# hygenie1228/PoseRisk_RELEASE

Measured on AMD Instinct MI355X. Metric: frames/sec (224x224 crops) through SPIN ResNet-50 + regressor + SMPL LBS + REBA/RULA, higher is better.
Workload: dtype f32; 1 GPU; configs[1]: batch=64 random 224x224 crops per GPU, ResNet-50+SMPL fp32; global_batch=64, batches_in_flight=3, hipgraph_replay=False, exchange=none, dist_world_size=1

## Files before the change

### poserisk_release_amd/csrc/conv_fused.hip

```cpp
#include <cstdlib>

#include "conv_igemm.h"
#include "kernel_vocab.h"

namespace pr {
namespace {

constexpr int BK = kConvBK;

struct FArgs {
  const float* x;
  const float* w2;
  const float* bias2;
  const float* w3;
  const float* bias3;
  const float* res;
  float* y;
  unsigned x_bytes, w2_bytes, w3_bytes;
  int H, W, Cin, log2Cin, HoWo, M, nk, N3, relu3;
};

constexpr int kStage = 2 * 64 * 128;
constexpr int kT2 = 0;
constexpr int kRing = 2 * 8192;
constexpr int kLds = 2 * kStage;

__global__ __launch_bounds__(256, 5) void conv3x3_conv1x1_f32(const FArgs a) {
#if defined(__HIP_DEVICE_COMPILE__)
  extern __shared__ __attribute__((aligned(16))) char smem[];
  const int nb = gridDim.x, bid = blockIdx.x;
  const int tile_m = xcd_contiguous_block<int>(bid, nb);
  const int m0 = tile_m * 64;
  const int tid = threadIdx.x, lane = tid & 63;
  const int wave = __builtin_amdgcn_readfirstlane(tid >> 6);
  const int wm = wave >> 1, wn = wave & 1;

  const int q = PR_DMA_SWIZZLE_SLOT(lane, wave);
  const auto xsrc = make_rsrc(a.x, (int)a.x_bytes);
  const auto w2src = make_rsrc(a.w2, (int)a.w2_bytes);
  const auto w3src = make_rsrc(a.w3, (int)a.w3_bytes);
  int a_base[2], a_hi0[2], a_wi0[2];
  unsigned b2_off[2], b3_off[2];
  const int K2 = a.nk * BK;
#pragma unroll
  for (int i = 0; i < 2; ++i) {
    const int r = 8 * (wave + 4 * i) + (lane >> 3);
    const int m = m0 + r;
    if (m < a.M) {
      const int img = m / a.HoWo, rem = m - img * a.HoWo;
      const int ho = rem / a.W, wo = rem - ho * a.W;
      a_hi0[i] = ho - 1;
      a_wi0[i] = wo - 1;
      a_base[i] = (((img * a.H + a_hi0[i]) * a.W + a_wi0[i]) * a.Cin + q * 4) * 4;
    } else {
      a_hi0[i] = -(1 << 28);
      a_wi0[i] = 0;
      a_base[i] = (int)kOOB;
    }
    b2_off[i] = (unsigned)((r * K2 + q * 4) * 4);
    b3_off[i] = (unsigned)((r * 64 + q * 4) * 4);
  }

  auto issue = [&](int kt, int buf) {
    char* stage = smem + buf * kStage;
    const int k0 = kt * BK;
    const int tap = k0 >> a.log2Cin, ci0 = k0 & (a.Cin - 1);
    const int kh = tap / 3, kw = tap - kh * 3;
    const int koff = ((kh * a.W + kw) * a.Cin + ci0) * 4;
#pragma unroll
    for (int i = 0; i < 2; ++i) {
      const bool ok = (unsigned)(a_hi0[i] + kh) < (unsigned)a.H && (unsigned)(a_wi0[i] + kw) < (unsigned)a.W;
      __builtin_amdgcn_raw_ptr_buffer_load_lds(xsrc, (lds_void*)(stage + (wave + 4 * i) * 1024), 16,
                                               ok ? (unsigned)(a_base[i] + koff) : kOOB, 0, 0, 0);
    }
#pragma unroll
    for (int i = 0; i < 2; ++i)
      __builtin_amdgcn_raw_ptr_buffer_load_lds(w2src, (lds_void*)(stage + 8192 + (wave + 4 * i) * 1024), 16, b2_off[i],
                                               kt * 128, 0, 0);
  };
  auto issue3 = [&](int s) {
    char* stage = smem + kRing + (s & 1) * 8192;
    const int soff = ((s >> 1) * 64 * 64 + (s & 1) * BK) * 4;
#pragma unroll
    for (int i = 0; i < 2; ++i)
      __builtin_amdgcn_raw_ptr_buffer_load_lds(w3src, (lds_void*)(stage + (wave + 4 * i) * 1024), 16, b3_off[i], soff, 0, 0);
  };

  const int frow = lane & 31, fh = lane >> 5, fsw = (frow >> 1) & 7;
  int foff[BK / 8];
#pragma unroll
  for (int kk = 0; kk < BK / 8; ++kk) foff[kk] = frow * 128 + (((2 * kk + fh) ^ fsw) << 4);

  f32x16 acc;
#pragma unroll
  for (int e = 0; e < 16; ++e) acc[e] = 0.f;
  auto compute = [&](const char* Ab, const char* Bb) {
    f32x4 af[BK / 8], bf[BK / 8];
#pragma unroll
    for (int kk = 0; kk < BK / 8; ++kk) {
      af[kk] = *reinterpret_cast<const f32x4*>(Ab + foff[kk]);
      bf[kk] = *reinterpret_cast<const f32x4*>(Bb + foff[kk]);
    }
    __builtin_amdgcn_sched_barrier(0);
#pragma unroll
    for (int kk = 0; kk < BK / 8; ++kk)
#pragma unroll
      for (int j = 0; j < 4; ++j) acc = __builtin_amdgcn_mfma_f32_32x32x2f32(af[kk][j], bf[kk][j], acc, 0, 0, 0);
  };

  issue(0, 0);
  for (int kt = 0; kt < a.nk; ++kt) {
    asm volatile("s_waitcnt vmcnt(0)" ::: "memory");
    __builtin_amdgcn_s_barrier();
    asm volatile("" ::: "memory");
    if (kt + 1 < a.nk) issue(kt + 1, (kt + 1) & 1);
    const char* st = smem + (kt & 1) * kStage;
    compute(st + wm * 32 * 128, st + 8192 + wn * 32 * 128);
  }

  __syncthreads();
  issue3(0);
  {
    const int c = lane & 31;
    const float b2 = a.bias2[wn * 32 + c];
    char* t2 = smem + kT2 + wn * 8192;
#pragma unroll
    for (int e = 0; e < 16; ++e) {
      const int r = wm * 32 + 4 * (lane >> 5) + (e & 3) + 8 * (e >> 2);
      const float v = fmaxf(acc[e] + b2, 0.f);
      *reinterpret_cast<float*>(t2 + r * 128 + ((((c >> 2) ^ ((r >> 1) & 7))) << 4) + (c & 3) * 4) = v;
    }
  }

  const int nsteps = (a.N3 >> 6) * 2;
  float rfrag[16];
  const int col_l = lane & 31, row_h = 4 * (lane >> 5);
  const int yz_bytes = a.M * a.N3 * 4;
  const auto rsrc = make_rsrc(a.res ? a.res : a.y, yz_bytes);
  const auto ysrc = make_rsrc(a.y, yz_bytes);
  const int frag_off = ((m0 + wm * 32 + row_h) * a.N3 + wn * 32 + col_l) * 4;
  const int mlim = a.M - (m0 + wm * 32 + row_h);
  for (int s = 0; s < nsteps; ++s) {
    asm volatile("s_waitcnt vmcnt(0) lgkmcnt(0)" ::: "memory");
    __builtin_amdgcn_s_barrier();
    asm volatile("" ::: "memory");
    if (s + 1 < nsteps) issue3(s + 1);
    const int n0 = (s >> 1) * 64;
    if ((s & 1) == 0) {
#pragma unroll
      for (int e = 0; e < 16; ++e) acc[e] = 0.f;
      if (a.res) {
#pragma unroll
        for (int e = 0; e < 16; ++e)
          rfrag[e] = __builtin_bit_cast(float, __builtin_amdgcn_raw_buffer_load_b32(
                                                   rsrc, (e & 3) + 8 * (e >> 2) < mlim ? frag_off : (int)kOOB,
                                                   (n0 + ((e & 3) + 8 * (e >> 2)) * a.N3) * 4, 0));
      }
    }
    compute(smem + kT2 + (s & 1) * 8192 + wm * 32 * 128, smem + kRing + (s & 1) * 8192 + wn * 32 * 128);
    if (s & 1) {
      const float b3 = a.bias3[n0 + wn * 32 + col_l];
#pragma unroll
      for (int e = 0; e < 16; ++e) {
        float v = acc[e] + b3;
        if (a.res) v += rfrag[e];
        if (a.relu3) v = fmaxf(v, 0.f);
        __builtin_amdgcn_raw_buffer_store_b32(__builtin_bit_cast(unsigned, v), ysrc,
                                              (e & 3) + 8 * (e >> 2) < mlim ? frag_off : (int)kOOB,
                                              (n0 + ((e & 3) + 8 * (e >> 2)) * a.N3) * 4, 0);
      }
    }
  }
#endif
}

struct PArgs {
  const float* x;
  const float* x2;
  const float* w;
  const float* bias;
  const float* res;
  float* y;
  unsigned x_bytes, x2_bytes, w_bytes;
  int M, N, K, nk, nk1, HoWo, Wo, H2, W2, Cin2, stride2;
  int chunks, nsplit, relu;
};

template <bool DUAL>
__global__ __launch_bounds__(256, 3) void conv1x1_panel_f32(const PArgs a) {
#if defined(__HIP_DEVICE_COMPILE__)
  extern __shared__ __attribute__((aligned(16))) char smem[];
  const int nb = gridDim.x, bid = blockIdx.x;
  const int item = xcd_contiguous_block<int>(bid, nb);
  const int panel = item / a.nsplit, part = item - panel * a.nsplit;
  const int m0 = panel * 64, nbase = part * a.chunks * 64;
  const int tid = threadIdx.x, lane = tid & 63;
  const int wave = __builtin_amdgcn_readfirstlane(tid >> 6);
  const int wm = wave >> 1, wn = wave & 1;
  const int q = PR_DMA_SWIZZLE_SLOT(lane, wave);
  const auto xsrc = make_rsrc(a.x, (int)a.x_bytes);
  [[maybe_unused]] const auto x2src = make_rsrc(DUAL ? a.x2 : a.x, DUAL ? (int)a.x2_bytes : 0);
  const auto wsrc = make_rsrc(a.w, (int)a.w_bytes);
  char* ring = smem + a.nk * 8192;

  const int K1 = a.nk1 * BK;
  unsigned b_off[2];
#pragma unroll
  for (int i = 0; i < 2; ++i) {
    const int r = 8 * (wave + 4 * i) + (lane >> 3);
    const int m = m0 + r;
    unsigned base = kOOB, base2 = kOOB;
    if (m < a.M) {
      base = (unsigned)((m * K1 + q * 4) * 4);
      if (DUAL) {
        const int img = m / a.HoWo, rem = m - img * a.HoWo;
        const int ho = rem / a.Wo, wo = rem - ho * a.Wo;
        base2 = (unsigned)((((img * a.H2 + ho * a.stride2) * a.W2 + wo * a.stride2) * a.Cin2 + q * 4) * 4);
      }
    }
    for (int kt = 0; kt < a.nk; ++kt) {
      lds_void* dst = (lds_void*)(smem + kt * 8192 + (wave + 4 * i) * 1024);
      if (DUAL && kt >= a.nk1) __builtin_amdgcn_raw_ptr_buffer_load_lds(x2src, dst, 16, base2, (kt - a.nk1) * 128, 0, 0);
      else __builtin_amdgcn_raw_ptr_buffer_load_lds(xsrc, dst, 16, base, kt * 128, 0, 0);
    }
    b_off[i] = (unsigned)((r * a.K + q * 4) * 4);
  }
  auto issue_w = [&](int chunk, int kt, int buf) {
    const int soff = ((nbase + chunk * 64) * a.K + kt * BK) * 4;
#pragma unroll
    for (int i = 0; i < 2; ++i)
      __builtin_amdgcn_raw_ptr_buffer_load_lds(wsrc, (lds_void*)(ring + buf * 8192 + (wave + 4 * i) * 1024), 16, b_off[i],
                                               soff, 0, 0);
  };
  issue_w(0, 0, 0);

  const int frow = lane & 31, fh = lane >> 5, fsw = (frow >> 1) & 7;
  int foff[BK / 8];
#pragma unroll
  for (int kk = 0; kk < BK / 8; ++kk) foff[kk] = frow * 128 + (((2 * kk + fh) ^ fsw) << 4);
  f32x16 acc;
  float rfrag[16];
  const int col_l = lane & 31, row_h = 4 * (lane >> 5);
  const int yz_bytes = a.M * a.N * 4;
  const auto rsrc = make_rsrc(a.res ? a.res : a.y, yz_bytes);
  const auto ysrc = make_rsrc(a.y, yz_bytes);
  const int frag_off = ((m0 + wm * 32 + row_h) * a.N + nbase + wn * 32 + col_l) * 4;
  const int mlim = a.M - (m0 + wm * 32 + row_h);

  int chunk = 0, kt = 0;
  const int nsteps = a.chunks * a.nk;
  for (int s = 0; s < nsteps; ++s) {
    asm volatile("s_waitcnt vmcnt(0)" ::: "memory");
    __builtin_amdgcn_s_barrier();
    asm volatile("" ::: "memory");
    {
      int nchunk = chunk, nkt = kt + 1;
      if (nkt == a.nk) { nkt = 0; ++nchunk; }
      if (s + 1 < nsteps) issue_w(nchunk, nkt, (s + 1) & 1);
    }
    const int n0 = chunk * 64;
    if (kt == 0) {
#pragma unroll
      for (int e = 0; e < 16; ++e) acc[e] = 0.f;
      if (a.res) {
#pragma unroll
        for (int e = 0; e < 16; ++e)
          rfrag[e] = __builtin_bit_cast(float, __builtin_amdgcn_raw_buffer_load_b32(
                                                   rsrc, (e & 3) + 8 * (e >> 2) < mlim ? frag_off : (int)kOOB,
                                                   (n0 + ((e & 3) + 8 * (e >> 2)) * a.N) * 4, 0));
      }
    }
    {
      const char* Ab = smem + kt * 8192 + wm * 32 * 128;
      const char* Bb = ring + (s & 1) * 8192 + wn * 32 * 128;
      f32x4 af[BK / 8], bf[BK / 8];
#pragma unroll
      for (int kk = 0; kk < BK / 8; ++kk) {
        af[kk] = *reinterpret_cast<const f32x4*>(Ab + foff[kk]);
        bf[kk] = *reinterpret_cast<const f32x4*>(Bb + foff[kk]);
      }
      __builtin_amdgcn_sched_barrier(0);
#pragma unroll
      for (int kk = 0; kk < BK / 8; ++kk)
#pragma unroll
        for (int j = 0; j < 4; ++j) acc = __builtin_amdgcn_mfma_f32_32x32x2f32(af[kk][j], bf[kk][j], acc, 0, 0, 0);
    }
    if (kt == a.nk - 1) {
      const float b = a.bias ? a.bias[nbase + n0 + wn * 32 + col_l] : 0.f;
#pragma unroll
      for (int e = 0; e < 16; ++e) {
        float v = acc[e] + b;
        if (a.res) v += rfrag[e];
        if (a.relu) v = fmaxf(v, 0.f);
        __builtin_amdgcn_raw_buffer_store_b32(__builtin_bit_cast(unsigned, v), ysrc,
                                              (e & 3) + 8 * (e >> 2) < mlim ? frag_off : (int)kOOB,
                                              (n0 + ((e & 3) + 8 * (e >> 2)) * a.N) * 4, 0);
      }
      kt = 0;
      ++chunk;
    } else {
      ++kt;
    }
  }
#endif
}


struct FArgsB {
  const unsigned short* x;
  const unsigned short* w2;
  const float* bias2;
  const unsigned short* w3;
  const float* bias3;
  const unsigned short* res;
  unsigned short* y;
  unsigned x_bytes, w2_bytes, w3_bytes;
  int H, W, Cin, log2Cin, HoWo, M, nk, N3, relu3;
};

constexpr int kBStage = 2 * 64 * 128;
constexpr int kBT2 = 0;
constexpr int kBRing = 8192;
constexpr int kBCt = 8192 + 16384;
constexpr int kBLds = kBCt + 64 * 64 * 4;

__device__ inline unsigned short f2bf(float f) {
  const __bf16 h = (__bf16)f;
  return __builtin_bit_cast(unsigned short, h);
}

__global__ __launch_bounds__(256, 4) void conv3x3_conv1x1_bf16(const FArgsB a) {
#if defined(__HIP_DEVICE_COMPILE__)
  extern __shared__ __attribute__((aligned(16))) char smem[];
  constexpr int BKB = 64;
  const int nb = gridDim.x, bid = blockIdx.x;
  const int tile_m = xcd_contiguous_block<int>(bid, nb);
  const int m0 = tile_m * 64;
  const int tid = threadIdx.x, lane = tid & 63;
  const int wave = __builtin_amdgcn_readfirstlane(tid >> 6);
  const int wm = wave >> 1, wn = wave & 1;
  const int q = PR_DMA_SWIZZLE_SLOT(lane, wave);
  const auto xsrc = make_rsrc(a.x, (int)a.x_bytes);
  const auto w2src = make_rsrc(a.w2, (int)a.w2_bytes);
  const auto w3src = make_rsrc(a.w3, (int)a.w3_bytes);
  int a_base[2], a_hi0[2], a_wi0[2];
  unsigned b2_off[2], b3_off[2];
  const int K2 = a.nk * BKB;
#pragma unroll
  for (int i = 0; i < 2; ++i) {
    const int r = 8 * (wave + 4 * i) + (lane >> 3);
    const int m = m0 + r;
    if (m < a.M) {
      const int img = m / a.HoWo, rem = m - img * a.HoWo;
      const int ho = rem / a.W, wo = rem - ho * a.W;
      a_hi0[i] = ho - 1;
      a_wi0[i] = wo - 1;
      a_base[i] = (((img * a.H + a_hi0[i]) * a.W + a_wi0[i]) * a.Cin + q * 8) * 2;
    } else {
      a_hi0[i] = -(1 << 28);
      a_wi0[i] = 0;
      a_base[i] = (int)kOOB;
    }
    b2_off[i] = (unsigned)((r * K2 + q * 8) * 2);
    b3_off[i] = (unsigned)((r * 64 + q * 8) * 2);
  }
  auto issue = [&](int kt, int buf) {
    char* stage = smem + buf * kBStage;
    const int tap = kt % 9, ci0 = (kt / 9) * BKB;
    const int kh = tap / 3, kw = tap - kh * 3;
    const int koff = ((kh * a.W + kw) * a.Cin + ci0) * 2;
#pragma unroll
    for (int i = 0; i < 2; ++i) {
      const bool ok = (unsigned)(a_hi0[i] + kh) < (unsigned)a.H && (unsigned)(a_wi0[i] + kw) < (unsigned)a.W;
      __builtin_amdgcn_raw_ptr_buffer_load_lds(xsrc, (lds_void*)(stage + (wave + 4 * i) * 1024), 16,
                                               ok ? (unsigned)(a_base[i] + koff) : kOOB, 0, 0, 0);
    }
#pragma unroll
    for (int i = 0; i < 2; ++i)
      __builtin_amdgcn_raw_ptr_buffer_load_lds(w2src, (lds_void*)(stage + 8192 + (wave + 4 * i) * 1024), 16, b2_off[i],
                                               kt * 128, 0, 0);
  };
  auto issue3 = [&](int nc) {
    char* stage = smem + kBRing + (nc & 1) * 8192;
#pragma unroll
    for (int i = 0; i < 2; ++i)
      __builtin_amdgcn_raw_ptr_buffer_load_lds(w3src, (lds_void*)(stage + (wave + 4 * i) * 1024), 16, b3_off[i],
                                               nc * 64 * 64 * 2, 0, 0);
  };

  const int frow = lane & 31, fh = lane >> 5, fsw = (frow >> 1) & 7;
  int foff[4];
#pragma unroll
  for (int kk = 0; kk < 4; ++kk) foff[kk] = frow * 128 + (((2 * kk + fh) ^ fsw) << 4);
  f32x16 acc;
#pragma unroll
  for (int e = 0; e < 16; ++e) acc[e] = 0.f;
  auto compute = [&](const char* Ab, const char* Bb) {
    bf16x8 af[4], bf[4];
#pragma unroll
    for (int kk = 0; kk < 4; ++kk) {
      af[kk] = *reinterpret_cast<const bf16x8*>(Ab + foff[kk]);
      bf[kk] = *reinterpret_cast<const bf16x8*>(Bb + foff[kk]);
    }
#pragma unroll
    for (int kk = 0; kk < 4; ++kk) acc = mfma_bf16_step(af[kk], bf[kk], acc);
  };

  issue(0, 0);
  for (int kt = 0; kt < a.nk; ++kt) {
    asm volatile("s_waitcnt vmcnt(0)" ::: "memory");
    __builtin_amdgcn_s_barrier();
    asm volatile("" ::: "memory");
    if (kt + 1 < a.nk) issue(kt + 1, (kt + 1) & 1);
    const char* st = smem + (kt & 1) * kBStage;
    compute(st + wm * 32 * 128, st + 8192 + wn * 32 * 128);
  }

  __syncthreads();
  issue3(0);
  {
    const int c = wn * 32 + (lane & 31);
    const float b2 = a.bias2[c];
    char* t2 = smem + kBT2;
#pragma unroll
    for (int e = 0; e < 16; ++e) {
      const int r = wm * 32 + 4 * (lane >> 5) + (e & 3) + 8 * (e >> 2);
      *reinterpret_cast<unsigned short*>(t2 + r * 128 + ((((c >> 3) ^ ((r >> 1) & 7))) << 4) + (c & 7) * 2) =
          f2bf(fmaxf(acc[e] + b2, 0.f));
    }
  }

  float* Ct = reinterpret_cast<float*>(smem + kBCt);
  const int nchunks = a.N3 >> 6;
  u16x8 rpre[2];
  for (int nc = 0; nc < nchunks; ++nc) {
    asm volatile("s_waitcnt vmcnt(0) lgkmcnt(0)" ::: "memory");
    __builtin_amdgcn_s_barrier();
    asm volatile("" ::: "memory");
    if (nc + 1 < nchunks) issue3(nc + 1);
    const int n0 = nc * 64;
    if (a.res) {
#pragma unroll
      for (int i = 0; i < 2; ++i) {
        const int idx = tid + i * 256;
        const int r = idx >> 3, cc = idx & 7;
        const int row = m0 + r;
        const u16x8 z = {0, 0, 0, 0, 0, 0, 0, 0};
        rpre[i] = row < a.M ? *reinterpret_cast<const u16x8*>(a.res + (long)row * a.N3 + n0 + cc * 8) : z;
      }
    }
#pragma unroll
    for (int e = 0; e < 16; ++e) acc[e] = 0.f;
    compute(smem + kBT2 + wm * 32 * 128, smem + kBRing + (nc & 1) * 8192 + wn * 32 * 128);
    {
      const int col_l = lane & 31, row_h = 4 * (lane >> 5);
#pragma unroll
// ... 25 lines not shown
#endif
}

struct PArgsB {
  const unsigned short* x;
  const unsigned short* x2;
  const unsigned short* w;
  const float* bias;
  const unsigned short* res;
  unsigned short* y;
  unsigned x_bytes, x2_bytes, w_bytes;
  int M, N, K, nk, nk1, HoWo, Wo, H2, W2, Cin2, stride2;
  int chunks, nsplit, relu;
};

template <bool DUAL>
__global__ __launch_bounds__(256, 2) void conv1x1_panel_bf16(const PArgsB a) {
#if defined(__HIP_DEVICE_COMPILE__)
  extern __shared__ __attribute__((aligned(16))) char smem[];
  constexpr int BKB = 64;
  const int nb = gridDim.x, bid = blockIdx.x;
  const int item = xcd_contiguous_block<int>(bid, nb);
  const int panel = item / a.nsplit, part = item - panel * a.nsplit;
  const int m0 = panel * 64, nbase = part * a.chunks * 64;
  const int tid = threadIdx.x, lane = tid & 63;
  const int wave = __builtin_amdgcn_readfirstlane(tid >> 6);
  const int wm = wave >> 1, wn = wave & 1;
  const int q = PR_DMA_SWIZZLE_SLOT(lane, wave);
  const auto xsrc = make_rsrc(a.x, (int)a.x_bytes);
  [[maybe_unused]] const auto x2src = make_rsrc(DUAL ? a.x2 : a.x, DUAL ? (int)a.x2_bytes : 0);
  const auto wsrc = make_rsrc(a.w, (int)a.w_bytes);
  char* ring = smem + a.nk * 8192;
  float* Ct = reinterpret_cast<float*>(ring + 16384);

  const int K1 = a.nk1 * BKB;
  unsigned b_off[2];
#pragma unroll
  for (int i = 0; i < 2; ++i) {
    const int r = 8 * (wave + 4 * i) + (lane >> 3);
    const int m = m0 + r;
    unsigned base = kOOB, base2 = kOOB;
    if (m < a.M) {
      base = (unsigned)((m * K1 + q * 8) * 2);
      if (DUAL) {
        const int img = m / a.HoWo, rem = m - img * a.HoWo;
        const int ho = rem / a.Wo, wo = rem - ho * a.Wo;
        base2 = (unsigned)((((img * a.H2 + ho * a.stride2) * a.W2 + wo * a.stride2) * a.Cin2 + q * 8) * 2);
      }
    }
    for (int kt = 0; kt < a.nk; ++kt) {
      lds_void* dst = (lds_void*)(smem + kt * 8192 + (wave + 4 * i) * 1024);
      if (DUAL && kt >= a.nk1) __builtin_amdgcn_raw_ptr_buffer_load_lds(x2src, dst, 16, base2, (kt - a.nk1) * 128, 0, 0);
      else __builtin_amdgcn_raw_ptr_buffer_load_lds(xsrc, dst, 16, base, kt * 128, 0, 0);
    }
    b_off[i] = (unsigned)((r * a.K + q * 8) * 2);
  }
  auto issue_w = [&](int chunk, int kt, int buf) {
    const int soff = ((nbase + chunk * 64) * a.K + kt * BKB) * 2;
#pragma unroll
    for (int i = 0; i < 2; ++i)
      __builtin_amdgcn_raw_ptr_buffer_load_lds(wsrc, (lds_void*)(ring + buf * 8192 + (wave + 4 * i) * 1024), 16, b_off[i],
                                               soff, 0, 0);
  };
  issue_w(0, 0, 0);

  const int frow = lane & 31, fh = lane >> 5, fsw = (frow >> 1) & 7;
  int foff[4];
#pragma unroll
  for (int kk = 0; kk < 4; ++kk) foff[kk] = frow * 128 + (((2 * kk + fh) ^ fsw) << 4);
  f32x16 acc;
  u16x8 rpre[2];
  int chunk = 0, kt = 0;
  const int nsteps = a.chunks * a.nk;
  for (int s = 0; s < nsteps; ++s) {
    asm volatile("s_waitcnt vmcnt(0)" ::: "memory");
    __builtin_amdgcn_s_barrier();
    asm volatile("" ::: "memory");
    {
      int nchunk = chunk, nkt = kt + 1;
      if (nkt == a.nk) { nkt = 0; ++nchunk; }
      if (s + 1 < nsteps) issue_w(nchunk, nkt, (s + 1) & 1);
    }
    const int n0 = nbase + chunk * 64;
    if (kt == 0) {
#pragma unroll
      for (int e = 0; e < 16; ++e) acc[e] = 0.f;
      if (a.res) {
#pragma unroll
        for (int i = 0; i < 2; ++i) {
          const int idx = tid + i * 256;
          const int r = idx >> 3, cc = idx & 7;
          const int row = m0 + r;
          const u16x8 z = {0, 0, 0, 0, 0, 0, 0, 0};
          rpre[i] = row < a.M ? *reinterpret_cast<const u16x8*>(a.res + (long)row * a.N + n0 + cc * 8) : z;
        }
      }
    }
    {
      const char* Ab = smem + kt * 8192 + wm * 32 * 128;
      const char* Bb = ring + (s & 1) * 8192 + wn * 32 * 128;
      bf16x8 af[4], bf[4];
#pragma unroll
      for (int kk = 0; kk < 4; ++kk) {
        af[kk] = *reinterpret_cast<const bf16x8*>(Ab + foff[kk]);
        bf[kk] = *reinterpret_cast<const bf16x8*>(Bb + foff[kk]);
      }
#pragma unroll
      for (int kk = 0; kk < 4; ++kk) acc = mfma_bf16_step(af[kk], bf[kk], acc);
    }
    if (kt == a.nk - 1) {
      {
        const int col_l = lane & 31, row_h = 4 * (lane >> 5);
#pragma unroll
        for (int e = 0; e < 16; ++e) Ct[(wm * 32 + row_h + (e & 3) + 8 * (e >> 2)) * 64 + wn * 32 + col_l] = acc[e];
      }
      __syncthreads();
#pragma unroll
      for (int i = 0; i < 2; ++i) {
        const int idx = tid + i * 256;
        const int r = idx >> 3, cc = idx & 7;
        const int row = m0 + r, col = n0 + cc * 8;
        if (row >= a.M) continue;
        const f32x4 v0 = *reinterpret_cast<const f32x4*>(&Ct[r * 64 + cc * 8]);
        const f32x4 v1 = *reinterpret_cast<const f32x4*>(&Ct[r * 64 + cc * 8 + 4]);
        float v[8] = {v0[0], v0[1], v0[2], v0[3], v1[0], v1[1], v1[2], v1[3]};
        if (a.bias) {
          const f32x4 b0 = *reinterpret_cast<const f32x4*>(a.bias + col);
          const f32x4 b1 = *reinterpret_cast<const f32x4*>(a.bias + col + 4);
#pragma unroll
          for (int e = 0; e < 4; ++e) {
            v[e] += b0[e];
            v[4 + e] += b1[e];
          }
        }
        if (a.res) {
#pragma unroll
          for (int e = 0; e < 8; ++e) v[e] += __uint_as_float((unsigned)rpre[i][e] << 16);
        }
        u16x8 out;
#pragma unroll
        for (int e = 0; e < 8; ++e) out[e] = f2bf(a.relu ? fmaxf(v[e], 0.f) : v[e]);
        *reinterpret_cast<u16x8*>(a.y + (long)row * a.N + col) = out;
      }
      kt = 0;
      ++chunk;
    } else {
      ++kt;
    }
  }
#endif
}

}

int conv_fused3_launch(const ConvProblem& p, hipStream_t stream) {
  PR_REQUIRE(p.KH == 3 && p.KW == 3 && p.stride == 1 && p.pad == 1 && p.Cout == 64 && p.Ho == p.H && p.Wo == p.W,
             "conv_fused3: the first convolution must be 3x3 / stride 1 / pad 1 with 64 output channels");
  const int l2 = ilog2_exact(p.Cin);
  PR_REQUIRE(l2 >= 0 && p.Cin % (p.precision == 1 ? 64 : BK) == 0, "conv_fused3: Cin must be a power of two >= %d (%d)",
             p.precision == 1 ? 64 : BK, p.Cin);
  PR_REQUIRE(p.w3 && p.bias && p.bias3 && p.y3 && p.N3 > 0 && p.N3 % 64 == 0 && !p.x2 && p.groups == 1,
             "conv_fused3: needs both biases, W3 and an output with N3 %% 64 == 0 (%d)", p.N3);
  const size_t xb = (size_t)p.B * p.H * p.W * p.Cin * (p.precision == 1 ? 2 : 4);
  PR_REQUIRE(xb < (1ull << 31) && (size_t)p.M() * p.N3 * 4 < (1ull << 31), "conv_fused3: tensor too large for one launch");
  if (p.precision == 1) {
    FArgsB fb;
    const int Kp = conv_kpad_bf16(p.K());
    fb.x = reinterpret_cast<const unsigned short*>(p.x); fb.w2 = reinterpret_cast<const unsigned short*>(p.w);
    fb.bias2 = p.bias; fb.w3 = reinterpret_cast<const unsigned short*>(p.w3); fb.bias3 = p.bias3;
    fb.res = reinterpret_cast<const unsigned short*>(p.res3); fb.y = reinterpret_cast<unsigned short*>(p.y3);
    fb.x_bytes = (unsigned)xb; fb.w2_bytes = (unsigned)((size_t)64 * Kp * 2); fb.w3_bytes = (unsigned)((size_t)p.N3 * 64 * 2);
    fb.H = p.H; fb.W = p.W; fb.Cin = p.Cin; fb.log2Cin = l2; fb.HoWo = p.H * p.W; fb.M = p.M(); fb.nk = Kp / 64;
    fb.N3 = p.N3; fb.relu3 = p.relu3;
    if (fb.M == 0) return PR_OK;
    hipLaunchKernelGGL(conv3x3_conv1x1_bf16, dim3(ceil_div(fb.M, 64)), dim3(256), kBLds, stream, fb);
    return check_launch("conv3x3_conv1x1_bf16");
  }
  FArgs fa;
  fa.x = p.x; fa.w2 = p.w; fa.bias2 = p.bias; fa.w3 = p.w3; fa.bias3 = p.bias3; fa.res = p.res3; fa.y = p.y3;
  fa.x_bytes = (unsigned)xb; fa.w2_bytes = (unsigned)((size_t)64 * p.Kpad() * 4); fa.w3_bytes = (unsigned)((size_t)p.N3 * 64 * 4);
  fa.H = p.H; fa.W = p.W; fa.Cin = p.Cin; fa.log2Cin = l2; fa.HoWo = p.H * p.W; fa.M = p.M(); fa.nk = p.Kpad() / BK;
  fa.N3 = p.N3; fa.relu3 = p.relu3;
  if (fa.M == 0) return PR_OK;
  hipLaunchKernelGGL(conv3x3_conv1x1_f32, dim3(ceil_div(fa.M, 64)), dim3(256), kLds, stream, fa);
  return check_launch("conv3x3_conv1x1_f32");
}

int conv_panel_launch(const ConvProblem& p, hipStream_t stream) {
  const int K2 = p.x2 ? p.Cin2 : 0, K = p.Cin + K2;
  const int bk = p.precision == 1 ? 64 : BK, el = p.precision == 1 ? 2 : 4, kmax = p.precision == 1 ? 512 : 256;
  PR_REQUIRE(p.KH == 1 && p.KW == 1 && p.stride == 1 && p.pad == 0 && p.groups == 1 && !p.w3,
             "conv_panel: 1x1 / stride-1 convolutions only");
  PR_REQUIRE(p.Cin % bk == 0 && K2 % bk == 0 && K <= kmax && p.Cout % 64 == 0,
             "conv_panel: K %d (<= %d, multiple of %d), N %d", K, kmax, bk, p.Cout);
  const size_t xb = (size_t)p.M() * p.Cin * el, x2b = p.x2 ? (size_t)p.B * p.H2 * p.W2 * p.Cin2 * el : 0;
  PR_REQUIRE(xb < (1ull << 31) && x2b < (1ull << 31) && (size_t)p.M() * p.Cout * 4 < (1ull << 31),
             "conv_panel: tensor too large for one launch");
  if (p.x2)
    PR_REQUIRE((p.H2 - 1) / p.stride2 + 1 == p.Ho && (p.W2 - 1) / p.stride2 + 1 == p.Wo,
               "conv_panel: second source %dx%d / stride %d does not land on the %dx%d output", p.H2, p.W2, p.stride2, p.Ho, p.Wo);
  if (p.precision == 1) {
    PArgsB pb;
    pb.x = reinterpret_cast<const unsigned short*>(p.x); pb.x2 = reinterpret_cast<const unsigned short*>(p.x2);
    pb.w = reinterpret_cast<const unsigned short*>(p.w); pb.bias = p.bias;
    pb.res = reinterpret_cast<const unsigned short*>(p.res); pb.y = reinterpret_cast<unsigned short*>(p.y);
    pb.x_bytes = (unsigned)xb; pb.x2_bytes = (unsigned)x2b; pb.w_bytes = (unsigned)((size_t)p.Cout * K * 2);
    pb.M = p.M(); pb.N = p.Cout; pb.K = K; pb.nk = K / 64; pb.nk1 = p.Cin / 64;
    pb.HoWo = p.Ho * p.Wo; pb.Wo = p.Wo; pb.H2 = p.H2; pb.W2 = p.W2; pb.Cin2 = p.Cin2; pb.stride2 = p.stride2;
    pb.relu = p.relu;
    if (pb.M == 0) return PR_OK;
    const int panels = ceil_div(pb.M, 64), nchunks = p.Cout / 64;
    const int nsplit = conv_panel_nsplit(panels, nchunks);
    pb.nsplit = nsplit;
    pb.chunks = nchunks / nsplit;
    const size_t lds = (size_t)pb.nk * 8192 + 16384 + 16384, lds_max = (size_t)(kmax / bk) * 8192 + 16384 + 16384;
    if (p.x2) {
      static std::atomic<uint64_t> attr_done{0};
      PR_TRY(ensure_dynamic_lds(reinterpret_cast<const void*>(conv1x1_panel_bf16<true>), lds_max, attr_done));
      hipLaunchKernelGGL(conv1x1_panel_bf16<true>, dim3(panels * nsplit), dim3(256), lds, stream, pb);
    } else {
      static std::atomic<uint64_t> attr_done{0};
      PR_TRY(ensure_dynamic_lds(reinterpret_cast<const void*>(conv1x1_panel_bf16<false>), lds_max, attr_done));
      hipLaunchKernelGGL(conv1x1_panel_bf16<false>, dim3(panels * nsplit), dim3(256), lds, stream, pb);
    }
    return check_launch("conv1x1_panel_bf16");
  }
  PArgs pa;
  pa.x = p.x; pa.x2 = p.x2; pa.w = p.w; pa.bias = p.bias; pa.res = p.res; pa.y = p.y;
  pa.x_bytes = (unsigned)xb; pa.x2_bytes = (unsigned)x2b; pa.w_bytes = (unsigned)((size_t)p.Cout * K * 4);
  pa.M = p.M(); pa.N = p.Cout; pa.K = K; pa.nk = K / BK; pa.nk1 = p.Cin / BK;
  pa.HoWo = p.Ho * p.Wo; pa.Wo = p.Wo; pa.H2 = p.H2; pa.W2 = p.W2; pa.Cin2 = p.Cin2; pa.stride2 = p.stride2;
  pa.relu = p.relu;
  if (pa.M == 0) return PR_OK;
  const int panels = ceil_div(pa.M, 64), nchunks = p.Cout / 64;
  const int nsplit = conv_panel_nsplit(panels, nchunks);
  pa.nsplit = nsplit;
  pa.chunks = nchunks / nsplit;
  const size_t lds = (size_t)pa.nk * 8192 + 16384, lds_max = (size_t)(kmax / bk) * 8192 + 16384;
  if (p.x2) {
    static std::atomic<uint64_t> attr_done{0};
    PR_TRY(ensure_dynamic_lds(reinterpret_cast<const void*>(conv1x1_panel_f32<true>), lds_max, attr_done));
    hipLaunchKernelGGL(conv1x1_panel_f32<true>, dim3(panels * nsplit), dim3(256), lds, stream, pa);
  } else {
    static std::atomic<uint64_t> attr_done{0};
    PR_TRY(ensure_dynamic_lds(reinterpret_cast<const void*>(conv1x1_panel_f32<false>), lds_max, attr_done));
    hipLaunchKernelGGL(conv1x1_panel_f32<false>, dim3(panels * nsplit), dim3(256), lds, stream, pa);
  }
  return check_launch("conv1x1_panel_f32");
}

}
```

Before: 17790 frames/s.

## Software-pipeline fused conv3x3+1x1 kernel with interleaved DMA, LDS reads and epilogue

Adds a pipelined variant of the fused conv3x3→conv1x1 kernel. It interleaves the global→LDS DMA for step k+2 and the LDS fragment reads for step k+1 between the MFMAs of step k. The 1x1 tail is rewritten to double-buffer accumulators, overlapping stores and residual loads for the previous chunk with the current chunk's compute. The aim is to hide memory and barrier latency behind matrix ops, at the cost of lower occupancy (4 waves per SIMD bound) and more registers. A pipelined panel path and timing instrumentation are also added, but the panel path is disabled by default.

```diff
diff --git a/poserisk_release_amd/csrc/conv_fused.hip b/poserisk_release_amd/csrc/conv_fused.hip
--- a/poserisk_release_amd/csrc/conv_fused.hip
+++ b/poserisk_release_amd/csrc/conv_fused.hip
@@ -1,12 +1,30 @@
 #include <cstdlib>
+#include <type_traits>
 
 #include "conv_igemm.h"
 #include "kernel_vocab.h"
+#include "timing_hooks.h"
 
 namespace pr {
 namespace {
 
 constexpr int BK = kConvBK;
+#if defined(PR_EXPERIMENT) && (PR_EXPERIMENT >= 11 && PR_EXPERIMENT <= 14)
+constexpr bool kOldFusedLoop = PR_EXPERIMENT == 11 || PR_EXPERIMENT == 13;
+constexpr bool kOldPanelLoop = PR_EXPERIMENT == 11 || PR_EXPERIMENT == 14;
+#else
+constexpr bool kOldFusedLoop = false;
+constexpr bool kOldPanelLoop = true;
+#endif
+
+#ifdef PR_TIMING_HOOKS
+#define PR_TL_EXP(x, bit) ((x) & (bit))
+#define PR_TL_STAMP(st, k) \
+  if ((st) && threadIdx.x == 0) (st)[(size_t)blockIdx.x * 8 + (k)] = __builtin_amdgcn_s_memrealtime()
+#else
+#define PR_TL_EXP(x, bit) 0
+#define PR_TL_STAMP(st, k)
+#endif
 
 struct FArgs {
   const float* x;
@@ -18,16 +36,207 @@
   float* y;
   unsigned x_bytes, w2_bytes, w3_bytes;
   int H, W, Cin, log2Cin, HoWo, M, nk, N3, relu3;
+  int exp;
+  unsigned long long* stamps;
 };
 
 constexpr int kStage = 2 * 64 * 128;
-constexpr int kT2 = 0;
-constexpr int kRing = 2 * 8192;
+[[maybe_unused]] constexpr int kT2 = 0;
+[[maybe_unused]] constexpr int kRing = 2 * 8192;
 constexpr int kLds = 2 * kStage;
-
-__global__ __launch_bounds__(256, 5) void conv3x3_conv1x1_f32(const FArgs a) {
+#ifndef PR_FUSED_PIPE_WAVES
+#define PR_FUSED_PIPE_WAVES 4
+#endif
+constexpr int kFusedPipeWgPerSimd = PR_FUSED_PIPE_WAVES;
+
+struct TailFrags {
+  f32x4 a[BK / 8], b[BK / 8];
+};
+
+struct Tail {
+  const char* a_lds;
+  char* ring;
+  const char* b_rows;
+  unsigned w_off[2];
+  int w_soff;
+  int w_chunk;
+  int nk, chunks;
+  int N4;
+  int col4;
+  int frag_off, mlim;
+  int bias_voff;
+  int wave;
+  bool has_res, relu;
+  int exp;
+  unsigned long long* stamps;
+};
+
+__device__ __forceinline__ u32x4 rsrc_words(const void* p, unsigned bytes) {
+  const unsigned long long v = (unsigned long long)p;
+  return u32x4{(unsigned)v, (unsigned)(v >> 32) & 0xffffu, bytes, (unsigned)kBufferRsrcFlags};
+}
+__device__ __forceinline__ void load_b32_uncounted(float& dst, const u32x4 rsrc, int voff, int soff) {
+  asm volatile("buffer_load_dword %0, %1, %2, %3 offen" : "+v"(dst) : "v"(voff), "s"(rsrc), "s"(soff) : "memory");
+}
+
+template <bool NK2, typename Rsrc, typename BeforeWait>
+__device__ __forceinline__ void tail_walk(const Tail& t, const Rsrc wsrc, const Rsrc ysrc, const u32x4 res_words,
+                                          const u32x4 bias_words, const int (&foff)[BK / 8], BeforeWait&& before_wait) {
+  using P0 = std::integral_constant<int, 0>;
+  using P1 = std::integral_constant<int, 1>;
+  const int nk = NK2 ? 2 : t.nk;
+  const int nsteps = t.chunks * nk;
+  const bool bare = PR_TL_EXP(t.exp, 8);
+
+  auto dma = [&](int chunk, int kt, int buf, int piece) {
+    __builtin_amdgcn_raw_ptr_buffer_load_lds(wsrc, (lds_void*)(t.ring + buf * 8192 + (t.wave + 4 * piece) * 1024), 16,
+                                             t.w_off[piece], t.w_soff + chunk * t.w_chunk + kt * 128, 0, 0);
+  };
+  auto read_piece = [&](int kt, int buf, int piece, TailFrags& f) {
+    const int kk = piece >> 1;
+    if ((piece & 1) == 0) f.a[kk] = *reinterpret_cast<const f32x4*>(t.a_lds + kt * 8192 + foff[kk]);
+    else f.b[kk] = *reinterpret_cast<const f32x4*>(t.b_rows + buf * 8192 + foff[kk]);
+  };
+
+  f32x16 acc0, acc1;
+  float prv[16], bias0 = 0.f, bias1 = 0.f;
+#pragma unroll
+  for (int e = 0; e < 16; ++e) acc0[e] = acc1[e] = prv[e] = 0.f;
+
+  auto item_voff = [&](int e) {
+    int ml = t.mlim;
+    asm volatile("" : "+v"(ml));
+    return (e & 3) + 8 * (e >> 2) < ml ? t.frag_off : (int)kOOB;
+  };
+  auto item_soff = [&](int chunk, int e) { return t.col4 + chunk * 256 + ((e & 3) + 8 * (e >> 2)) * t.N4; };
+  auto out_item = [&](int chunk, int e, int voff, f32x16& acc, const float& bias) {
+    float v = acc[e] + bias;
+    if (t.has_res) v += prv[e];
+    if (t.relu) v = fmaxf(v, 0.f);
+    if (!PR_TL_EXP(t.exp, 1))
+      __builtin_amdgcn_raw_buffer_store_b32(__builtin_bit_cast(unsigned, v), ysrc, voff, item_soff(chunk, e), 0);
+    acc[e] = 0.f;
+  };
+  auto res_item = [&](int chunk, int e, int voff) {
+    if (!PR_TL_EXP(t.exp, 4)) load_b32_uncounted(prv[e], res_words, voff, item_soff(chunk, e));
+  };
+
+  auto step = [&](auto par_c, auto items_c, int c, int kt, const TailFrags& cur, TailFrags& nxt, f32x16& acc, f32x16& pacc,
+                  float& bias, const float& pbias) {
+    constexpr int PAR = decltype(par_c)::value, ITEMS = decltype(items_c)::value;
+    const int s = c * nk + kt;
+    const bool do_dma = s + 2 < nsteps && !bare, do_out = c > 0;
+    const int kt1 = kt + 1 < nk ? kt + 1 : 0;
+    const int c2 = kt + 2 < nk ? c : c + 1, kt2 = kt + 2 < nk ? kt + 2 : kt + 2 - nk;
+    if (!bare) {
+      asm volatile("s_waitcnt lgkmcnt(0)" ::: "memory");
+      __builtin_amdgcn_s_barrier();
+      asm volatile("" ::: "memory");
+    }
+    int n = 0;
+#pragma unroll
+    for (int kk = 0; kk < BK / 8; ++kk)
+#pragma unroll
+      for (int j = 0; j < 4; ++j) {
+        acc = __builtin_amdgcn_mfma_f32_32x32x2f32(cur.a[kk][j], cur.b[kk][j], acc, 0, 0, 0);
+        __builtin_amdgcn_sched_barrier(0);
+        if (n < 2) {
+          if (do_dma) dma(c2, kt2, PAR, n);
+          __builtin_amdgcn_sched_barrier(0);
+        } else if (n < 10) {
+          if (!bare) read_piece(kt1, PAR ^ 1, n - 2, nxt);
+          __builtin_amdgcn_sched_barrier(0);
+          if (ITEMS < 2 && !bare) {
+            const int e = 8 * ITEMS + n - 2, voff = item_voff(e);
+            if (do_out) out_item(c - 1, e, voff, pacc, pbias);
+            __builtin_amdgcn_sched_barrier(0);
+            res_item(c, e, voff);
+            __builtin_amdgcn_sched_barrier(0);
+          }
+        } else if (n == 10 && ITEMS == 0 && !bare) {
+          load_b32_uncounted(bias, bias_words, t.bias_voff, t.col4 + c * 256);
+          __builtin_amdgcn_sched_barrier(0);
+        }
+        ++n;
+      }
+  };
+  constexpr int kYoung0 = 9, kYoung1 = 8;
+  using I0 = std::integral_constant<int, 0>;
+  using I1 = std::integral_constant<int, 1>;
+  using I2 = std::integral_constant<int, 2>;
+  TailFrags f0, f1;
+  auto chunk = [&](int c, f32x16& acc, f32x16& pacc, float& bias, const float& pbias) {
+    if (!bare) {
+      if (c > 0 && nk == 2) asm volatile("s_waitcnt vmcnt(%0)" ::"n"(kYoung1) : "memory");
+      else asm volatile("s_waitcnt vmcnt(0)" ::: "memory");
+    }
+    step(P0{}, I0{}, c, 0, f0, f1, acc, pacc, bias, pbias);
+    if (!bare) asm volatile("s_waitcnt vmcnt(%0)" ::"n"(kYoung0) : "memory");
+    step(P1{}, I1{}, c, 1, f1, f0, acc, pacc, bias, pbias);
+    if constexpr (!NK2) {
+      for (int kt = 2; kt < nk; kt += 2) {
+        if (!bare) {
+          if (kt == 2) asm volatile("s_waitcnt vmcnt(%0)" ::"n"(kYoung1) : "memory");
+          else asm volatile("s_waitcnt vmcnt(0)" ::: "memory");
+        }
+        step(P0{}, I2{}, c, kt, f0, f1, acc, pacc, bias, pbias);
+        if (!bare) asm volatile("s_waitcnt vmcnt(0)" ::: "memory");
+        step(P1{}, I2{}, c, kt + 1, f1, f0, acc, pacc, bias, pbias);
+      }
+    }
+    if (c < 3) { PR_TL_STAMP(t.stamps, 2 + c); }
+  };
+
+  if (!bare) {
+    dma(0, 0, 0, 0);
+    dma(0, 0, 0, 1);
+    dma(0, 1, 1, 0);
+    dma(0, 1, 1, 1);
+  }
+  before_wait();
+  if (!bare) {
+    asm volatile("s_waitcnt vmcnt(2) lgkmcnt(0)" ::: "memory");
+    __builtin_amdgcn_s_barrier();
+    asm volatile("" ::: "memory");
+  }
+#pragma unroll
+  for (int pc = 0; pc < 8; ++pc) read_piece(0, 0, pc, f0);
+#ifdef PR_TIMING_HOOKS
+  if (bare) {
+#pragma unroll
+    for (int kk = 0; kk < BK / 8; ++kk) asm volatile("" : "+v"(f0.a[kk]), "+v"(f0.b[kk]), "+v"(f1.a[kk]), "+v"(f1.b[kk]));
+  }
+#endif
+  for (int c = 0; c < t.chunks; c += 2) {
+    chunk(c, acc0, acc1, bias0, bias1);
+    if (c + 1 < t.chunks) chunk(c + 1, acc1, acc0, bias1, bias0);
+  }
+  asm volatile("s_waitcnt vmcnt(0)" ::: "memory");
+  if (!bare) {
+    if (t.chunks & 1) {
+#pragma unroll
+      for (int e = 0; e < 16; ++e) out_item(t.chunks - 1, e, item_voff(e), acc0, bias0);
+    } else {
+#pragma unroll
+      for (int e = 0; e < 16; ++e) out_item(t.chunks - 1, e, item_voff(e), acc1, bias1);
+    }
+  }
+#ifdef PR_TIMING_HOOKS
+  if (bare) asm volatile("" ::"v"(acc0), "v"(acc1));
+  PR_TL_STAMP(t.stamps, 5);
+  asm volatile("s_waitcnt vmcnt(0)" ::: "memory");
+  PR_TL_STAMP(t.stamps, 6);
+#endif
+}
+
+template <bool PIPE>
+__global__ __launch_bounds__(256, PIPE ? kFusedPipeWgPerSimd : 5) void conv3x3_conv1x1_f32(const FArgs a) {
 #if defined(__HIP_DEVICE_COMPILE__)
   extern __shared__ __attribute__((aligned(16))) char smem[];
+  PR_TL_STAMP(a.stamps, 0);
+#ifdef PR_TIMING_HOOKS
+  if (a.stamps && threadIdx.x == 0) a.stamps[(size_t)blockIdx.x * 8 + 7] = __builtin_amdgcn_s_getreg(4 | (0 << 6) | (31 << 11));
+#endif
   const int nb = gridDim.x, bid = blockIdx.x;
   const int tile_m = xcd_contiguous_block<int>(bid, nb);
   const int m0 = tile_m * 64;
@@ -94,10 +303,16 @@
   f32x16 acc;
 #pragma unroll
   for (int e = 0; e < 16; ++e) acc[e] = 0.f;
-  auto compute = [&](const char* Ab, const char* Bb) {
+  auto compute = [&](const char* Ab, const char* Bb, [[maybe_unused]] bool bare = false) {
     f32x4 af[BK / 8], bf[BK / 8];
 #pragma unroll
     for (int kk = 0; kk < BK / 8; ++kk) {
+#ifdef PR_TIMING_HOOKS
+      if (bare) {
+        asm volatile("" : "=v"(af[kk]), "=v"(bf[kk]));
+        continue;
+      }
+#endif
       af[kk] = *reinterpret_cast<const f32x4*>(Ab + foff[kk]);
       bf[kk] = *reinterpret_cast<const f32x4*>(Bb + foff[kk]);
     }
@@ -108,6 +323,13 @@
       for (int j = 0; j < 4; ++j) acc = __builtin_amdgcn_mfma_f32_32x32x2f32(af[kk][j], bf[kk][j], acc, 0, 0, 0);
   };
 
+  [[maybe_unused]] float b2_early = 0.f;
+  if constexpr (PIPE) {
+    b2_early = a.bias2[wn * 32 + (lane & 31)];
+    asm volatile("" : "+v"(b2_early));
+  }
+
+  if (!PIPE || (a.nk & 1)) {
   issue(0, 0);
   for (int kt = 0; kt < a.nk; ++kt) {
     asm volatile("s_waitcnt vmcnt(0)" ::: "memory");
@@ -117,12 +339,73 @@
     const char* st = smem + (kt & 1) * kStage;
     compute(st + wm * 32 * 128, st + 8192 + wn * 32 * 128);
   }
+  } else {
+    using P0 = std::integral_constant<int, 0>;
+    using P1 = std::integral_constant<int, 1>;
+    auto issue_piece = [&](int kt, int buf, int piece) {
+      char* stage = smem + buf * kStage;
+      if (piece >= 2) {
+        const int i = piece - 2;
+        __builtin_amdgcn_raw_ptr_buffer_load_lds(w2src, (lds_void*)(stage + 8192 + (wave + 4 * i) * 1024), 16, b2_off[i], kt * 128,
+                                                 0, 0);
+        return;
+      }
+      const int i = piece, k0 = kt * BK;
+      const int tap = k0 >> a.log2Cin, ci0 = k0 & (a.Cin - 1);
+      const int kh = tap / 3, kw = tap - kh * 3;
+      const int koff = ((kh * a.W + kw) * a.Cin + ci0) * 4;
+      const bool ok = (unsigned)(a_hi0[i] + kh) < (unsigned)a.H && (unsigned)(a_wi0[i] + kw) < (unsigned)a.W;
+      __builtin_amdgcn_raw_ptr_buffer_load_lds(xsrc, (lds_void*)(stage + (wave + 4 * i) * 1024), 16,
+                                               ok ? (unsigned)(a_base[i] + koff) : kOOB, 0, 0, 0);
+    };
+    auto read_piece = [&](int buf, int piece, TailFrags& f) {
+      const int kk = piece >> 1;
+      const char* base = smem + buf * kStage;
+      if ((piece & 1) == 0) f.a[kk] = *reinterpret_cast<const f32x4*>(base + wm * 32 * 128 + foff[kk]);
+      else f.b[kk] = *reinterpret_cast<const f32x4*>(base + 8192 + wn * 32 * 128 + foff[kk]);
+    };
+    auto step = [&](auto par_c, int kt, bool do_dma, bool do_rd, const TailFrags& cur, TailFrags& nxt) {
+      constexpr int PAR = decltype(par_c)::value;
+      if (do_rd) asm volatile("s_waitcnt vmcnt(0)" ::: "memory");
+      asm volatile("s_waitcnt lgkmcnt(0)" ::: "memory");
+      __builtin_amdgcn_s_barrier();
+      asm volatile("" ::: "memory");
+      int n = 0;
+#pragma unroll
+      for (int kk = 0; kk < BK / 8; ++kk)
+#pragma unroll
+        for (int j = 0; j < 4; ++j) {
+          acc = __builtin_amdgcn_mfma_f32_32x32x2f32(cur.a[kk][j], cur.b[kk][j], acc, 0, 0, 0);
+          __builtin_amdgcn_sched_barrier(0);
+          if (n < 4) {
+            if (do_dma) issue_piece(kt + 2, PAR, n);
+            __builtin_amdgcn_sched_barrier(0);
+          } else if (n < 12) {
+            read_piece(PAR ^ 1, n - 4, nxt);
+            __builtin_amdgcn_sched_barrier(0);
+          }
+          ++n;
+        }
+    };
+    TailFrags f0, f1;
+    issue(0, 0);
+    issue(1, 1);
+    asm volatile("s_waitcnt vmcnt(4)" ::: "memory");
+    __builtin_amdgcn_s_barrier();
+    asm volatile("" ::: "memory");
+#pragma unroll
+    for (int pc = 0; pc < 8; ++pc) read_piece(0, pc, f0);
+    for (int kt = 0; kt < a.nk; kt += 2) {
+      step(P0{}, kt, kt + 2 < a.nk, true, f0, f1);
+      step(P1{}, kt + 1, kt + 3 < a.nk, kt + 2 < a.nk, f1, f0);
+    }
+  }
+  PR_TL_STAMP(a.stamps, 1);
 
   __syncthreads();
-  issue3(0);
-  {
+  auto write_t2 = [&]() {
     const int c = lane & 31;
-    const float b2 = a.bias2[wn * 32 + c];
+    const float b2 = PIPE ? b2_early : a.bias2[wn * 32 + c];
     char* t2 = smem + kT2 + wn * 8192;
 #pragma unroll
     for (int e = 0; e < 16; ++e) {
@@ -130,26 +413,49 @@
       const float v = fmaxf(acc[e] + b2, 0.f);
       *reinterpret_cast<float*>(t2 + r * 128 + ((((c >> 2) ^ ((r >> 1) & 7))) << 4) + (c & 3) * 4) = v;
     }
-  }
+  };
+  const int col_l = lane & 31, row_h = 4 * (lane >> 5);
+  const int yz_bytes = a.M * a.N3 * 4;
+  const auto ysrc = make_rsrc(a.y, yz_bytes);
+  const int mlim = a.M - (m0 + wm * 32 + row_h);
+  const int frag_off = ((m0 + wm * 32 + row_h) * a.N3 + wn * 32 + col_l) * 4;
+  if constexpr (PIPE) {
+    Tail t;
+    t.a_lds = smem + kT2 + wm * 32 * 128;
+    t.ring = smem + kRing;
+    t.b_rows = smem + kRing + wn * 32 * 128;
+    t.w_off[0] = b3_off[0]; t.w_off[1] = b3_off[1];
+    t.w_soff = 0; t.w_chunk = 64 * 64 * 4;
+    t.nk = 2; t.chunks = a.N3 >> 6;
+    t.N4 = a.N3 * 4; t.col4 = 0; t.frag_off = frag_off; t.mlim = mlim; t.bias_voff = (wn * 32 + col_l) * 4;
+    t.wave = wave; t.has_res = a.res != nullptr; t.relu = a.relu3 != 0; t.exp = a.exp; t.stamps = a.stamps;
+    tail_walk<true>(t, w3src, ysrc, rsrc_words(a.res, a.res ? (unsigned)yz_bytes : 0u), rsrc_words(a.bias3, (unsigned)a.N3 * 4u), foff,
+                    write_t2);
+    return;
+  }
+  issue3(0);
+  write_t2();
 
   const int nsteps = (a.N3 >> 6) * 2;
   float rfrag[16];
-  const int col_l = lane & 31, row_h = 4 * (lane >> 5);
-  const int yz_bytes = a.M * a.N3 * 4;
+#ifdef PR_TIMING_HOOKS
+#pragma unroll
+  for (int e = 0; e < 16; ++e) rfrag[e] = 0.f;
+#endif
+  const bool bare = PR_TL_EXP(a.exp, 8);
   const auto rsrc = make_rsrc(a.res ? a.res : a.y, yz_bytes);
-  const auto ysrc = make_rsrc(a.y, yz_bytes);
-  const int frag_off = ((m0 + wm * 32 + row_h) * a.N3 + wn * 32 + col_l) * 4;
-  const int mlim = a.M - (m0 + wm * 32 + row_h);
   for (int s = 0; s < nsteps; ++s) {
+    if (!bare || s == 0) {
     asm volatile("s_waitcnt vmcnt(0) lgkmcnt(0)" ::: "memory");
     __builtin_amdgcn_s_barrier();
     asm volatile("" ::: "memory");
-    if (s + 1 < nsteps) issue3(s + 1);
+    }
+    if (s + 1 < nsteps && !bare) issue3(s + 1);
     const int n0 = (s >> 1) * 64;
     if ((s & 1) == 0) {
 #pragma unroll
       for (int e = 0; e < 16; ++e) acc[e] = 0.f;
-      if (a.res) {
+      if (a.res && !PR_TL_EXP(a.exp, 4 | 8)) {
 #pragma unroll
         for (int e = 0; e < 16; ++e)
           rfrag[e] = __builtin_bit_cast(float, __builtin_amdgcn_raw_buffer_load_b32(
@@ -157,20 +463,30 @@
                                                    (n0 + ((e & 3) + 8 * (e >> 2)) * a.N3) * 4, 0));
       }
     }
-    compute(smem + kT2 + (s & 1) * 8192 + wm * 32 * 128, smem + kRing + (s & 1) * 8192 + wn * 32 * 128);
+    compute(smem + kT2 + (s & 1) * 8192 + wm * 32 * 128, smem + kRing + (s & 1) * 8192 + wn * 32 * 128, bare);
     if (s & 1) {
-      const float b3 = a.bias3[n0 + wn * 32 + col_l];
+      const float b3 = bare ? 0.f : a.bias3[n0 + wn * 32 + col_l];
 #pragma unroll
       for (int e = 0; e < 16; ++e) {
         float v = acc[e] + b3;
         if (a.res) v += rfrag[e];
         if (a.relu3) v = fmaxf(v, 0.f);
+        if (!PR_TL_EXP(a.exp, 1 | 8))
         __builtin_amdgcn_raw_buffer_store_b32(__builtin_bit_cast(unsigned, v), ysrc,
                                               (e & 3) + 8 * (e >> 2) < mlim ? frag_off : (int)kOOB,
                                               (n0 + ((e & 3) + 8 * (e >> 2)) * a.N3) * 4, 0);
       }
-    }
-  }
+#ifdef PR_TIMING_HOOKS
+      if (bare) asm volatile("" ::"v"(acc));
+      if ((s >> 1) < 3) { PR_TL_STAMP(a.stamps, 2 + (s >> 1)); }
+#endif
+    }
+  }
+#ifdef PR_TIMING_HOOKS
+  PR_TL_STAMP(a.stamps, 5);
+  asm volatile("s_waitcnt vmcnt(0)" ::: "memory");
+  PR_TL_STAMP(a.stamps, 6);
+#endif
 #endif
 }
 
@@ -184,12 +500,18 @@
   unsigned x_bytes, x2_bytes, w_bytes;
   int M, N, K, nk, nk1, HoWo, Wo, H2, W2, Cin2, stride2;
   int chunks, nsplit, relu;
+  int exp;
+  unsigned long long* stamps;
 };
 
-template <bool DUAL>
+template <bool DUAL, bool PIPE>
 __global__ __launch_bounds__(256, 3) void conv1x1_panel_f32(const PArgs a) {
 #if defined(__HIP_DEVICE_COMPILE__)
   extern __shared__ __attribute__((aligned(16))) char smem[];
+  PR_TL_STAMP(a.stamps, 0);
+#ifdef PR_TIMING_HOOKS
+  if (a.stamps && threadIdx.x == 0) a.stamps[(size_t)blockIdx.x * 8 + 7] = __builtin_amdgcn_s_getreg(4 | (0 << 6) | (31 << 11));
+#endif
   const int nb = gridDim.x, bid = blockIdx.x;
   const int item = xcd_contiguous_block<int>(bid, nb);
   const int panel = item / a.nsplit, part = item - panel * a.nsplit;
@@ -232,37 +554,60 @@
       __builtin_amdgcn_raw_ptr_buffer_load_lds(wsrc, (lds_void*)(ring + buf * 8192 + (wave + 4 * i) * 1024), 16, b_off[i],
                                                soff, 0, 0);
   };
-  issue_w(0, 0, 0);
-
+  PR_TL_STAMP(a.stamps, 1);
   const int frow = lane & 31, fh = lane >> 5, fsw = (frow >> 1) & 7;
   int foff[BK / 8];
 #pragma unroll
   for (int kk = 0; kk < BK / 8; ++kk) foff[kk] = frow * 128 + (((2 * kk + fh) ^ fsw) << 4);
+  const int col_l = lane & 31, row_h = 4 * (lane >> 5);
+  const int yz_bytes = a.M * a.N * 4;
+  const auto ysrc = make_rsrc(a.y, yz_bytes);
+  const int mlim = a.M - (m0 + wm * 32 + row_h);
+  if constexpr (PIPE) {
+    Tail t;
+    t.a_lds = smem + wm * 32 * 128;
+    t.ring = ring;
+    t.b_rows = ring + wn * 32 * 128;
+    t.w_off[0] = b_off[0]; t.w_off[1] = b_off[1];
+    t.w_soff = nbase * a.K * 4; t.w_chunk = 64 * a.K * 4;
+    t.nk = a.nk; t.chunks = a.chunks;
+    t.N4 = a.N * 4; t.col4 = nbase * 4; t.frag_off = ((m0 + wm * 32 + row_h) * a.N + wn * 32 + col_l) * 4; t.mlim = mlim;
+    t.bias_voff = (wn * 32 + col_l) * 4;
+    t.wave = wave; t.has_res = a.res != nullptr; t.relu = a.relu != 0; t.exp = a.exp; t.stamps = a.stamps;
+    tail_walk<false>(t, wsrc, ysrc, rsrc_words(a.res, a.res ? (unsigned)yz_bytes : 0u),
+                     rsrc_words(a.bias, a.bias ? (unsigned)a.N * 4u : 0u), foff, [] {});
+    return;
+  }
+  issue_w(0, 0, 0);
+
   f32x16 acc;
   float rfrag[16];
-  const int col_l = lane & 31, row_h = 4 * (lane >> 5);
-  const int yz_bytes = a.M * a.N * 4;
+#ifdef PR_TIMING_HOOKS
+#pragma unroll
+  for (int e = 0; e < 16; ++e) rfrag[e] = 0.f;
+#endif
+  const bool bare = PR_TL_EXP(a.exp, 8);
   const auto rsrc = make_rsrc(a.res ? a.res : a.y, yz_bytes);
-  const auto ysrc = make_rsrc(a.y, yz_bytes);
   const int frag_off = ((m0 + wm * 32 + row_h) * a.N + nbase + wn * 32 + col_l) * 4;
-  const int mlim = a.M - (m0 + wm * 32 + row_h);
 
   int chunk = 0, kt = 0;
   const int nsteps = a.chunks * a.nk;
   for (int s = 0; s < nsteps; ++s) {
+    if (!bare || s == 0) {
     asm volatile("s_waitcnt vmcnt(0)" ::: "memory");
     __builtin_amdgcn_s_barrier();
     asm volatile("" ::: "memory");
+    }
     {
       int nchunk = chunk, nkt = kt + 1;
       if (nkt == a.nk) { nkt = 0; ++nchunk; }
-      if (s + 1 < nsteps) issue_w(nchunk, nkt, (s + 1) & 1);
+      if (s + 1 < nsteps && !bare) issue_w(nchunk, nkt, (s + 1) & 1);
     }
     const int n0 = chunk * 64;
     if (kt == 0) {
 #pragma unroll
       for (int e = 0; e < 16; ++e) acc[e] = 0.f;
-      if (a.res) {
+      if (a.res && !PR_TL_EXP(a.exp, 4 | 8)) {
 #pragma unroll
         for (int e = 0; e < 16; ++e)
           rfrag[e] = __builtin_bit_cast(float, __builtin_amdgcn_raw_buffer_load_b32(
@@ -276,6 +621,12 @@
       f32x4 af[BK / 8], bf[BK / 8];
 #pragma unroll
       for (int kk = 0; kk < BK / 8; ++kk) {
+#ifdef PR_TIMING_HOOKS
+        if (bare) {
+          asm volatile("" : "=v"(af[kk]), "=v"(bf[kk]));
+          continue;
+        }
+#endif
         af[kk] = *reinterpret_cast<const f32x4*>(Ab + foff[kk]);
         bf[kk] = *reinterpret_cast<const f32x4*>(Bb + foff[kk]);
       }
@@ -286,22 +637,32 @@
         for (int j = 0; j < 4; ++j) acc = __builtin_amdgcn_mfma_f32_32x32x2f32(af[kk][j], bf[kk][j], acc, 0, 0, 0);
     }
     if (kt == a.nk - 1) {
-      const float b = a.bias ? a.bias[nbase + n0 + wn * 32 + col_l] : 0.f;
+      const float b = a.bias && !bare ? a.bias[nbase + n0 + wn * 32 + col_l] : 0.f;
 #pragma unroll
       for (int e = 0; e < 16; ++e) {
         float v = acc[e] + b;
         if (a.res) v += rfrag[e];
         if (a.relu) v = fmaxf(v, 0.f);
+        if (!PR_TL_EXP(a.exp, 1 | 8))
         __builtin_amdgcn_raw_buffer_store_b32(__builtin_bit_cast(unsigned, v), ysrc,
                                               (e & 3) + 8 * (e >> 2) < mlim ? frag_off : (int)kOOB,
                                               (n0 + ((e & 3) + 8 * (e >> 2)) * a.N) * 4, 0);
       }
+#ifdef PR_TIMING_HOOKS
+      if (bare) asm volatile("" ::"v"(acc));
+      if (chunk < 3) { PR_TL_STAMP(a.stamps, 2 + chunk); }
+#endif
       kt = 0;
       ++chunk;
     } else {
       ++kt;
     }
   }
+#ifdef PR_TIMING_HOOKS
+  PR_TL_STAMP(a.stamps, 5);
+  asm volatile("s_waitcnt vmcnt(0)" ::: "memory");
+  PR_TL_STAMP(a.stamps, 6);
+#endif
 #endif
 }
 
@@ -633,6 +994,13 @@
 }
 
 }
+
+#ifdef PR_TIMING_HOOKS
+static int tail_stamp_call() {
+  const char* e = getenv("POSERISK_TAIL_STAMP_CALL");
+  return e ? atoi(e) : 20;
+}
+#endif
 
 int conv_fused3_launch(const ConvProblem& p, hipStream_t stream) {
   PR_REQUIRE(p.KH == 3 && p.KW == 3 && p.stride == 1 && p.pad == 1 && p.Cout == 64 && p.Ho == p.H && p.Wo == p.W,
@@ -663,7 +1031,18 @@
   fa.H = p.H; fa.W = p.W; fa.Cin = p.Cin; fa.log2Cin = l2; fa.HoWo = p.H * p.W; fa.M = p.M(); fa.nk = p.Kpad() / BK;
   fa.N3 = p.N3; fa.relu3 = p.relu3;
   if (fa.M == 0) return PR_OK;
-  hipLaunchKernelGGL(conv3x3_conv1x1_f32, dim3(ceil_div(fa.M, 64)), dim3(256), kLds, stream, fa);
+  const int grid = ceil_div(fa.M, 64);
+  fa.exp = 0;
+  fa.stamps = nullptr;
+#ifdef PR_TIMING_HOOKS
+  if (const char* e = getenv("POSERISK_TAIL_EXP")) fa.exp = atoi(e);
+  if (fa.exp & 2) fa.w3_bytes = 0;
+  static int stamp_calls = 0;
+  StampRecorder stamp_rec("POSERISK_FUSED_STAMPS", (size_t)grid * 8, tail_stamp_call(), stamp_calls, stream);
+  fa.stamps = stamp_rec.stamps();
+#endif
+  if (kOldFusedLoop) hipLaunchKernelGGL(conv3x3_conv1x1_f32<false>, dim3(grid), dim3(256), kLds, stream, fa);
+  else hipLaunchKernelGGL(conv3x3_conv1x1_f32<true>, dim3(grid), dim3(256), kLds, stream, fa);
   return check_launch("conv3x3_conv1x1_f32");
 }
 
@@ -718,15 +1097,27 @@
   pa.nsplit = nsplit;
   pa.chunks = nchunks / nsplit;
   const size_t lds = (size_t)pa.nk * 8192 + 16384, lds_max = (size_t)(kmax / bk) * 8192 + 16384;
-  if (p.x2) {
-    static std::atomic<uint64_t> attr_done{0};
-    PR_TRY(ensure_dynamic_lds(reinterpret_cast<const void*>(conv1x1_panel_f32<true>), lds_max, attr_done));
-    hipLaunchKernelGGL(conv1x1_panel_f32<true>, dim3(panels * nsplit), dim3(256), lds, stream, pa);
-  } else {
-    static std::atomic<uint64_t> attr_done{0};
-    PR_TRY(ensure_dynamic_lds(reinterpret_cast<const void*>(conv1x1_panel_f32<false>), lds_max, attr_done));
-    hipLaunchKernelGGL(conv1x1_panel_f32<false>, dim3(panels * nsplit), dim3(256), lds, stream, pa);
-  }
+  const int grid = panels * nsplit;
+  pa.exp = 0;
+  pa.stamps = nullptr;
+#ifdef PR_TIMING_HOOKS
+  if (const char* e = getenv("POSERISK_TAIL_EXP")) pa.exp = atoi(e);
+  if (pa.exp & 2) pa.w_bytes = 0;
+  static int stamp_calls = 0;
+  StampRecorder stamp_rec("POSERISK_PANEL_STAMPS", (size_t)grid * 8, tail_stamp_call(), stamp_calls, stream);
+  pa.stamps = stamp_rec.stamps();
+#endif
+  const bool pipe = !kOldPanelLoop && pa.nk % 2 == 0;
+  auto go = [&](auto kern, std::atomic<uint64_t>& attr_done) -> int {
+    PR_TRY(ensure_dynamic_lds(reinterpret_cast<const void*>(kern), lds_max, attr_done));
+    hipLaunchKernelGGL(kern, dim3(grid), dim3(256), lds, stream, pa);
+    return PR_OK;
+  };
+  static std::atomic<uint64_t> attr_done[2][2] = {};
+  if (p.x2 && pipe) PR_TRY(go(conv1x1_panel_f32<true, true>, attr_done[1][1]));
+  else if (p.x2) PR_TRY(go(conv1x1_panel_f32<true, false>, attr_done[1][0]));
+  else if (pipe) PR_TRY(go(conv1x1_panel_f32<false, true>, attr_done[0][1]));
+  else PR_TRY(go(conv1x1_panel_f32<false, false>, attr_done[0][0]));
   return check_launch("conv1x1_panel_f32");
 }
 
```

After: 17840 frames/s (median of 6 runs). Within noise of the previous version (+0.3%).
